# introlab/rtabmap

Measured on AMD Instinct MI355X. Metric: loop-closure candidates/sec (49k vocab, 100k signatures, 500 desc/frame), higher is better.
Workload: dtype f32; 1 GPU; SURF-64 fp32 brute-force 2-NN (49k words) + NNDR + TF-IDF likelihood (100000 signatures x 500 words, Zipf), 500 desc/frame, 1 frame/step; world_size_observed=1, collective_backend=none, parallelism=1 GPU, last_frame_top_candidate_ok=True

## Files before the change

rtabmap_amd/csrc/engine.h:

```cpp
#pragma once
#include <hip/hip_runtime.h>
#include <stdint.h>
#include <algorithm>
#include <chrono>
#include <cmath>
#include <deque>
#include <string>
#include <thread>
#include <unordered_map>
#include <vector>

#include "../../include/lcd.h"
#include "devbuf.h"
#include "lcd_kernels.h"
#include "bayes.h"
#include "tfidf.h"

struct RowMirror {
    std::vector<int32_t> h_row_key;
    std::vector<char> h_row_live;
    bool rows_sorted = true;
    std::unordered_map<int32_t, int32_t> word_row;
    bool word_row_valid = false;
    int32_t next_word_id = 1;
// ... 206 lines not shown
    lcd::DevBuf d_queries, d_partial, d_knn_row, d_knn_word, d_knn_wslot, d_knn_dist, d_selfdist, d_out_word, d_out_wslot,
        d_n_new, d_tmp_i32, d_extra_rows, d_extra_id, d_extra_word, d_extra_dist, d_extra_row, d_like, d_slots, d_bits, row_norm, norm_max, d_partial2, d_partial3, d_fail_list, d_fail_count;
    lcd::DevBuf d_shard_selfdist;
    const void* shard_sd_desc = nullptr; int shard_sd_q = 0;
    bool fail_count_clean = false;
    bool bf_family() const { return knn_mode == 2 || knn_mode == 3; }
    int f16() const { return knn_mode == 3 ? 1 : 0; }
    int knn_mode = 2;
    bool hamming_mfma = false;
    bool wide_mfma = false;
    lcd::DevBuf d_wide_norm;
    int pipeline = 0;
    hipStream_t kst = nullptr;
    FramePipeline pipe;
    const void* last_fail_count = nullptr;
    AppendLog applog;
    int64_t vocab_capacity_cfg = 0;
    int64_t tail_filled_rows = 0;
    lcd::DevBuf d_rmlog;
    int64_t rm_seen = 0;
    bool rm_pending = false;
    int frames_since_reconcile = 0;
    int enqueue_clean(const int32_t* reg_cnt = nullptr);
    int reconcile();
    int32_t shard_first = 0, shard_block = 0;
    int shard_append = 0;
    int filter_units = -1;
    int strip_tiles = 0;
    lcd::PipeOpts popt;
    int sync_all();
// ... 35 lines not shown
```

rtabmap_amd/csrc/engine.hip:

```cpp
#include "engine_impl.h"
#include <dlfcn.h>

#include <algorithm>
#include <chrono>
#include <cmath>
#include <cstdlib>
#include <cstring>
#include <new>
#include <numeric>
#include <unordered_map>

using namespace lcd;

static_assert(sizeof(lcd::HypothesisOut) == sizeof(lcd_hypothesis), "lcd_hypothesis is the kernel's output record");

int RowMirror::find(int32_t word_id) {
    if (rows_sorted) {
        auto it = std::lower_bound(h_row_key.begin(), h_row_key.end(), word_id);
        if (it == h_row_key.end() || *it != word_id) return -1;
        const int r = (int)(it - h_row_key.begin());
        return h_row_live[r] ? r : -1;
    }
    if (!word_row_valid) {
        word_row.clear();
// ... 308 lines not shown
                                       h->d_knn_word.as<int32_t>(), h->d_knn_dist.as<float>(), h->d_bits.as<uint32_t>(), bw));
    }
    r->q = q;
    r->flags = (incremental ? LCD_Q_INCREMENTAL : 0) | (together ? LCD_Q_NEW_WORDS_COMPARED : 0);
    r->nndr = nndr;
    r->have_index = have_index;
    r->knn_word = h->d_knn_word.as<int32_t>();
    r->knn_dist = h->d_knn_dist.as<float>();
    r->selfdist = together ? h->d_selfdist.as<float>() : nullptr;
    r->ld = ld;
    r->cand_bits = together ? h->d_bits.as<uint32_t>() : nullptr;
    r->bw = bw;
    r->out_word = d_out_word;
    r->out_n_new = h->d_n_new.as<int32_t>();
    r->knn_row = h->d_knn_row.as<int32_t>();
    r->row_wslot = h->row_wslot.as<int32_t>();
    r->out_wslot = d_out_wslot;
    r->new_ws = WsRuns();
    r->cand_list = nullptr; r->cand_cnt = nullptr;
    if (side) {
        CandBits lay;
        cand_bits_layout(lay, h->d_bits.as<uint32_t>(), q, bw);
        r->cand_list = lay.list; r->cand_cnt = lay.cnt;
    }
    r->fail_count = nullptr;
    return LCD_OK;
}

extern "C" {

// ... 1341 lines not shown
```

rtabmap_amd/csrc/frame_pipeline.hip:

```cpp
#include "engine_impl.h"

#include <algorithm>
#include <chrono>
#include <cstring>

using namespace lcd;

namespace {
struct FrameHostTimer {
    lcd_engine* h; std::chrono::steady_clock::time_point t0;
    explicit FrameHostTimer(lcd_engine* e) : h(e), t0(std::chrono::steady_clock::now()) {}
    ~FrameHostTimer() { h->frame_host_ns += std::chrono::duration_cast<std::chrono::nanoseconds>(std::chrono::steady_clock::now() - t0).count(); h->frame_calls += 1; }
};
struct HostLap {
    lcd_engine* h; std::chrono::steady_clock::time_point t;
    explicit HostLap(lcd_engine* e) : h(e), t(std::chrono::steady_clock::now()) {}
    void lap(int i) { const auto n = std::chrono::steady_clock::now(); h->host_prof[i] += std::chrono::duration_cast<std::chrono::nanoseconds>(n - t).count(); t = n; }
};
struct FrameShape { bool incremental, together; int ld, bw; };
inline FrameShape frame_shape(const lcd_frame_args& a) {
    const bool incremental = (a.flags & LCD_Q_INCREMENTAL) != 0;
    const int ld = (a.q + 63) / 64 * 64;
    return FrameShape{incremental, incremental && (a.flags & LCD_Q_NEW_WORDS_COMPARED) != 0, ld, ld / 32};
}
// ... 153 lines not shown
        LCD_HIP(h, ring_reserve_grow(h, f.set, &FramePipeline::FrameScratch::d_partial3, knn_rowpar_partial_bytes((int)rows3, q),
                                     f.chained ? knn_rowpar_partial_bytes((int)std::min<int64_t>(rows3 + rows3 / 2 + 65536, 0x7FFFFF00ll), q) : 0));
    }
    k.vocab = h->vocab.p; k.vocab_bf = h->vocab_bf.p; k.row_norm = h->row_norm.as<float>(); k.norm_max_bits = h->norm_max.as<uint32_t>();
    k.row_id = h->row_id.as<int32_t>(); k.queries = a.d_descriptors; k.partial = sc.d_partial2.p;
    k.qsplit = sc.d_qsplit.p; k.qnorm = sc.d_qnorm.as<float>();
    k.out_row = sc.d_knn_row.as<int32_t>(); k.out_word = sc.d_knn_word.as<int32_t>(); k.out_dist = sc.d_knn_dist.as<float>();
    k.fail_list = sc.d_fail_list.as<int32_t>(); k.fail_count = sc.d_fail_count.as<int32_t>();
    k.n_lo = nullptr; k.n_hi = nullptr;
    if (f.chained) { k.n_lo = h->applog.count_after(f.vseq); k.n_hi = h->applog.count_before(f.vseq); }
    k.cb = CandBits();
    if (together) { k.cb.selfdist = sc.d_selfdist.as<float>(); k.cb.ld = ld; k.cb.nq = q; k.cb.have_index = 1; cand_bits_layout(k.cb, sc.d_bits.as<uint32_t>(), q, bw); }
    if (!sc.fail_count_clean) LCD_HIP(h, hipMemsetAsync(sc.d_fail_count.p, 0, 8, h->stream));
    sc.fail_count_clean = true;
    h->last_fail_count = sc.d_fail_count.p;
    ResolveArgs& r = f.r;
    r = ResolveArgs();
    r.q = q; r.flags = (incremental ? LCD_Q_INCREMENTAL : 0) | (together ? LCD_Q_NEW_WORDS_COMPARED : 0); r.nndr = a.nndr_ratio; r.have_index = 1;
    r.knn_word = k.out_word; r.knn_dist = k.out_dist; r.selfdist = together ? sc.d_selfdist.as<float>() : nullptr; r.ld = ld;
    r.cand_bits = together ? sc.d_bits.as<uint32_t>() : nullptr; r.bw = bw; r.out_word = a.d_word_ids; r.out_n_new = h->d_n_new.as<int32_t>();
    r.cand_list = together ? k.cb.list : nullptr; r.cand_cnt = together ? k.cb.cnt : nullptr;
    r.knn_row = k.out_row; r.row_wslot = h->row_wslot.as<int32_t>(); r.out_wslot = sc.d_out_wslot.as<int32_t>(); r.new_ws = WsRuns();
    r.fail_count = sc.d_fail_count.as<int32_t>();
    RowparArgs& rp = r.rp;
    rp.enabled = 1; rp.vocab = (const float*)h->vocab.p; rp.row_id = h->row_id.as<int32_t>(); rp.n_rows = (int)rows_bound;
    rp.n_rows_dev = k.n_hi;
    rp.queries = (const float*)a.d_descriptors; rp.fail_list = sc.d_fail_list.as<int32_t>(); rp.partial = (unsigned long long*)sc.d_partial3.p;
    rp.out_row = k.out_row; rp.out_word = k.out_word; rp.out_dist = k.out_dist;
    if (together) rp.cb = k.cb;
    return LCD_OK;
// ... 237 lines not shown

int lcd_frame_dev(lcd_engine* h, const lcd_frame_args* a) {
    LCD_TRY
    LCD_CHECK_HANDLE(h);
    FrameHostTimer timer__(h);
    lcd_engine::Range range__(h, "lcd_frame_dev");
    LCD_DEV_NODRAIN(h);
    return frame_dev_body(h, a);
    LCD_CATCH(h)
}

int lcd_debug_host_profile(const lcd_engine* h, int64_t* out9) {
    if (!h || !out9) return LCD_ERR_INVALID;
    for (int i = 0; i < 9; ++i) out9[i] = h->host_prof[i];
    return LCD_OK;
}

int lcd_slot_count(const lcd_engine* h, int64_t* n_slots) {
    if (!h || !n_slots) return LCD_ERR_INVALID;
    *n_slots = h->tfidf.n_slots + h->pipe.owed_sigs();
    return LCD_OK;
}

int lcd_frame_host(lcd_engine* h, const lcd_frame_host_args* a) {
    LCD_TRY
    LCD_CHECK_HANDLE(h);
    lcd_engine::Range range__(h, "lcd_frame_host");
    LCD_DEV(h);
    if (!a || a->struct_size != (int32_t)sizeof(lcd_frame_host_args)) return h->fail(LCD_ERR_INVALID, "lcd_frame_host: bad argument block");
    const int q = a->q;
// ... 47 lines not shown
```

rtabmap_amd/csrc/frame_tail_body.cuh:

```cuda
#pragma once
#include "tfidf.h"
#include "resolve_body.cuh"
#include "rowpar_body.cuh"

namespace lcd {
namespace {

template <typename T> __device__ __forceinline__ T gload(const T* p) { return *(const __attribute__((address_space(1))) T*)p; }
__device__ __forceinline__ uint2 gload2(const uint2* p) {
    const unsigned long long v = *(const __attribute__((address_space(1))) unsigned long long*)p;
    return make_uint2((uint32_t)v, (uint32_t)(v >> 32));
}

__device__ __forceinline__ uint4 gload4(const uint4* p) {
    typedef uint32_t u32x4 __attribute__((ext_vector_type(4)));
    const u32x4 v = *(const __attribute__((address_space(1))) u32x4*)p;
    return make_uint4(v.x, v.y, v.z, v.w);
}

__device__ __forceinline__ int32_t idf_to_fixed(float idf) {
    float s = idf * 67108864.0f;
    s = fminf(fmaxf(s, -2147483520.0f), 2147483520.0f);
    return (int32_t)rintf(s);
}
// ... 383 lines not shown
    else { asm volatile("" : "+v"(n_in_early), "+v"(ne0));
           fmask = resolve_body<NT>(ft_dyn_smem, r.q, r.flags, r.nndr, r.have_index, r.knn_word, r.knn_dist, r.selfdist, r.ld, r.cand_bits, r.bw, r.out_word,
                                    r.out_n_new, r.knn_row, r.row_wslot, r.out_wslot, r.new_ws); }
    if (threadIdx.x == 0 && r.fail_count) { r.fail_count[0] = 0; r.fail_count[1] = 0; r.fail_count[3] = 0; }
    if (r.ap.enabled) append_new_rows<NT>(r.ap, r.q, fmask, ft_dyn_smem + 2 * ((r.q + 63) / 64 * 2), r.new_ws, ft_dyn_smem + 2 * a.H + a.H / 64 + 8 + r.q,
                                          nullptr, 0, n_in_early);
    else append_pass_on(r.ap);
    FT_STAMP(1);
    retire_body(retire, a.slot_begin, a.slot_cnt, a.nw, a.slot_ni, a.slot_sig);
    __syncthreads();
    FT_STAMP(2);
    frame_words_body<NT, true>(ft_dyn_smem, a, lds_ws, have_ne0, ne0);
    FT_STAMP(3);
}

template <int NT>
__device__ __forceinline__ void frame_resolve_part(uint32_t* ft_dyn_smem, const ResolveArgs& r, int wb, int n_wb) {
    if (wb > 0) { rowpar_body<64, NT>(r.rp, wb - 1, n_wb - 1, r.fail_count); return; }
    constexpr int KPT = 1024 / NT;
    const bool fast = r.q <= KPT * NT;
    const bool helpers = r.rp.enabled && n_wb > 1;
    if (helpers && !fast) {
        if (threadIdx.x == 0 && r.fail_count[0] > 0) {
            while (__hip_atomic_load(&r.fail_count[3], __ATOMIC_RELAXED, __HIP_MEMORY_SCOPE_AGENT) == 0) __builtin_amdgcn_s_sleep(8);
            __builtin_amdgcn_fence(__ATOMIC_ACQUIRE, "agent");
        }
        __syncthreads();
    }
    int n_in_early = -1;
    const int32_t* cnt_in = (r.ap.enabled && r.ap.cnt_in) ? r.ap.cnt_in : nullptr;
    if (!fast && cnt_in) n_in_early = gload(cnt_in);
    FT_STAMP(0);
    const uint32_t* fmask;
    if (fast) fmask = resolve_body_fast<NT, KPT>(ft_dyn_smem, nullptr, r.q, r.flags, r.nndr, r.have_index, r.knn_word, r.knn_dist, r.selfdist,
                                                 r.ld, r.cand_bits, r.bw, r.out_word, r.out_n_new, r.knn_row, r.row_wslot, r.out_wslot, r.new_ws,
                                                 r.cand_list, r.cand_cnt, &n_in_early, cnt_in, helpers ? r.fail_count : nullptr, r.slots_are_rows != 0, r.straight != 0);
    else { asm volatile("" : "+v"(n_in_early)); fmask = resolve_body<NT>(ft_dyn_smem, r.q, r.flags, r.nndr, r.have_index, r.knn_word, r.knn_dist, r.selfdist, r.ld, r.cand_bits, r.bw, r.out_word,
                                  r.out_n_new, r.knn_row, r.row_wslot, r.out_wslot, r.new_ws, r.slots_are_rows != 0); }
    if (threadIdx.x == 0 && r.fail_count) { r.fail_count[0] = 0; r.fail_count[1] = 0; r.fail_count[3] = 0; }
    if (r.ap.enabled && r.ap.defer_rows) append_publish<NT>(r.ap, r.q, fmask, ft_dyn_smem + 2 * ((r.q + 63) / 64 * 2), n_in_early);
    else if (r.ap.enabled) {
        const int used = (3 * ((r.q + 63) / 64 * 2) + 4 + r.q + 3) & ~3;
        const int rows = (r.ap.lds_bytes / 4 - used) / 64;
        append_new_rows<NT>(r.ap, r.q, fmask, ft_dyn_smem + 2 * ((r.q + 63) / 64 * 2), r.new_ws, ft_dyn_smem + 3 * ((r.q + 63) / 64 * 2) + 4,
                            reinterpret_cast<float*>(ft_dyn_smem + used), rows > 0 ? (rows & ~3) : 0, n_in_early);
    } else append_pass_on(r.ap);
    FT_STAMP(1);
}
template <int NT>
__device__ __forceinline__ void frame_register_part_keys(uint32_t* ft_dyn_smem, const FwArgs& a, const RetireArgs& retire) {
    uint32_t ne0 = 0u;
    const bool have_ne0 = a.do_register && a.ne_counter != nullptr;
    if (threadIdx.x == 0 && have_ne0) ne0 = gload(a.ne_counter);
// ... 82 lines not shown
```

rtabmap_amd/csrc/knn_mfma_kernels.hip:

```cpp
#include <hip/hip_ext.h>
#include "lcd_kernels.h"
#include "rowpar_body.cuh"
#include "shard_body.cuh"
#include "frame_tail_body.cuh"
#include "score_body.cuh"

#include <algorithm>
#include <cstdlib>

namespace lcd {
namespace {

typedef float f32x16 __attribute__((ext_vector_type(16)));
constexpr int MF_BLOCK = 256;
constexpr int MF_WAVES = 4;
constexpr int MF_KEEP = 4;

__global__ void row_norm_kernel(const float* __restrict__ vocab, const int32_t* __restrict__ row_id, int first, int n, int dim,
                                float* __restrict__ aug, uint32_t* __restrict__ norm_max_bits) {
    const int r = first + blockIdx.x * blockDim.x + threadIdx.x;
    if (r >= first + n) return;
    float s = __int_as_float(0x7f800000);
    if (row_id[r] != 0) {
        s = 0.0f;
// ... 889 lines not shown
        static const hipError_t attrp1 = hipFuncSetAttribute(reinterpret_cast<const void*>(&frame_a_kernel_p<1>),
                                                             hipFuncAttributeMaxDynamicSharedMemorySize, (int)BF_LDS_BYTES_P);
        (void)attrp0; (void)attrp1;
        auto kern = f16 ? frame_a_kernel_p<1> : frame_a_kernel_p<0>;
        if (timed) hipExtLaunchKernelGGL(kern, dim3(grid), dim3(PIPE_BLOCK), (uint32_t)BF_LDS_BYTES_P, s, ev_begin, ev_end, 0u, f, px, tr, r, a, ret, qs);
        else kern<<<grid, PIPE_BLOCK, BF_LDS_BYTES_P, s>>>(f, px, tr, r, a, ret, qs);
    } else {
        auto kern = f16 ? frame_a_kernel<1> : frame_a_kernel<0>;
        if (timed) hipExtLaunchKernelGGL(kern, dim3(grid), dim3(PIPE_BLOCK), (uint32_t)BF_LDS_BYTES_Q, s, ev_begin, ev_end, 0u, f, tr, r, a, ret, qs);
        else kern<<<grid, PIPE_BLOCK, BF_LDS_BYTES_Q, s>>>(f, tr, r, a, ret, qs);
    }
    return hipGetLastError();
}


hipError_t launch_frame_b(const PipeKnn* k, const ScoreArgs* score, int score_wgs, hipStream_t s, hipEvent_t ev_begin, hipEvent_t ev_end,
                          const AppendRowsArgs* app, const PipeOpts& opt) {
    RerankArgs rk{};
    int n_rerank = 0;
    if (k) {
        const MfmaPlan& p = k->plan;
        uint64_t* pk = (uint64_t*)k->partial;
        rk.pk = pk; rk.pl = (uint32_t*)(pk + (size_t)(p.n_blocks > 0 ? p.n_blocks : 1) * BF_KEEP * p.qpad);
        rk.n_blocks = p.n_blocks; rk.nq = p.q; rk.vocab = (const float*)k->vocab; rk.queries = (const float*)k->queries; rk.row_id = k->row_id;
        rk.norm_max_bits = k->norm_max_bits; rk.out_row = k->out_row; rk.out_word = k->out_word; rk.out_dist = k->out_dist;
        rk.fail_list = k->fail_list; rk.fail_count = k->fail_count; rk.cb = k->cb; rk.n_lo = k->n_lo; rk.n_hi = k->n_hi; rk.plan_rows = p.n_rows; rk.f16 = p.f16;
        n_rerank = ((p.q + 1) / 2 + 7) & ~7;
    }
    ScoreArgs A{};
    if (score) A = *score; else score_wgs = 0;
    AppendRowsArgs ar{};
    int n_app = 0;
    if (app && app->ap.enabled && app->ap.defer_rows) { ar = *app; n_app = ar.n_wgs = APPEND_ROW_WGS; }
    if (n_rerank + score_wgs + n_app == 0) return hipSuccess;
    const uint32_t dyn = ((k && k->n_hi) || n_app) ? PIPE_B_STAGE_ROWS * 256u + 512u : 0u;
    rk.stage_rows = (dyn && k && k->n_hi) ? (int)PIPE_B_STAGE_ROWS : 0;
    ar.ap.lds_bytes = (int)(PIPE_B_STAGE_ROWS * 256u);
    if (k && n_app) { rk.pend_desc = ar.ap.descriptors; rk.pend_list = ar.ap.list_out; rk.pend_first_id = ar.ap.first_id; }
    if (k && n_app && opt.cross_frames && k->cross && k->cross_cols == (const void*)ar.ap.descriptors) { rk.cross = k->cross; rk.cross_ld = k->cross_ld; }
    const bool writers = opt.append_from_rerank == 0;
    if (!writers && k && n_app > 0 && k->n_hi && k->plan.q > 0 && rk.stage_rows >= 4) n_app = 0;
    const bool shadow = k && k->plan.n_shadow > 0 && k->sh_mask && k->sh_x && k->sh_q > 0 && app && app->ap.enabled && app->ap.defer_rows && rk.pend_desc && !rk.cross;
    if (k && k->plan.n_shadow > 0 && !shadow) return hipErrorInvalidValue;
    if (shadow) { rk.sh_mask = k->sh_mask; rk.sh_q = k->sh_q; rk.sh_x = k->sh_x; rk.sh_ld = k->sh_ld; }
    const int n_wr = (!writers && n_app == 0 && k && app && app->ap.enabled && app->ap.defer_rows && k->n_hi && k->plan.q > 0 && rk.stage_rows >= 4 && !rk.cross &&
                      (opt.row_writer_wgs > 0 || shadow)) ? (opt.row_writer_wgs > 0 ? opt.row_writer_wgs : 16) : 0;
    if (shadow && n_wr == 0) return hipErrorInvalidValue;
    const bool split = n_app > 0 && score && score->n_closed >= (opt.append_split_buckets >= 0 ? opt.append_split_buckets : APPEND_SPLIT_BUCKETS);
    if (split || n_app == 0) {
        if (n_rerank + score_wgs > 0) {
            if (ev_begin != nullptr && ev_end != nullptr)
                hipExtLaunchKernelGGL(frame_b_kernel<false>, dim3(n_rerank + n_wr + score_wgs), dim3(PIPE_B_BLOCK), dyn, s, ev_begin, ev_end, 0u, rk, n_rerank, A, score_wgs, ar, n_wr);
            else frame_b_kernel<false><<<n_rerank + n_wr + score_wgs, PIPE_B_BLOCK, dyn, s>>>(rk, n_rerank, A, score_wgs, ar, n_wr);
        }
        if (n_app > 0) append_rows_kernel<<<n_app, PIPE_B_BLOCK, PIPE_B_STAGE_ROWS * 256u, s>>>(ar);
        return hipGetLastError();
    }
    if (ev_begin != nullptr && ev_end != nullptr)
        hipExtLaunchKernelGGL(frame_b_kernel<true>, dim3(n_rerank + score_wgs + n_app), dim3(PIPE_B_BLOCK), dyn, s, ev_begin, ev_end, 0u, rk, n_rerank, A, score_wgs, ar, 0);
    else frame_b_kernel<true><<<n_rerank + score_wgs + n_app, PIPE_B_BLOCK, dyn, s>>>(rk, n_rerank, A, score_wgs, ar, 0);
    return hipGetLastError();
}

}

extern "C" int lcd_debug_frame_plan(int q, int n_rows, int new_words_compared, int* out) {
    if (q <= 0 || n_rows <= 0 || !out) return -1;
    const int tiles = new_words_compared ? lcd::knn_selfdist_wgs(q) : 0;
    const lcd::MfmaPlan p = lcd::knn_bf16_plan_pipelined(q, n_rows, tiles, -1);
    out[0] = p.tiles_per_block; out[1] = p.n_blocks; out[2] = lcd::bf16_persistent_px(p); out[3] = tiles; out[4] = (q + lcd::BF_QB - 1) / lcd::BF_QB;
    return 0;
}

extern "C" int lcd_debug_wide_mfma_plan(int q, int n_rows, int dim, int units, int* out9) {
    lcd::WidePlan p;
    if (!out9 || !lcd::knn_wide_mfma_plan(q, n_rows, dim, units, &p)) return -1;
    out9[0] = p.tiles_per_block; out9[1] = p.n_blocks; out9[2] = p.n_qblocks; out9[3] = p.group_q; out9[4] = p.qpad;
    out9[5] = (int)(lcd::knn_wide_partial_bytes(p) / 4); out9[6] = lcd::MF_STRIP_TILES;
    out9[7] = (p.tiles_per_block + lcd::MF_STRIP_TILES - 1) / lcd::MF_STRIP_TILES; out9[8] = p.n_wgs;
    return 0;
// ... 18 lines not shown
```

rtabmap_amd/csrc/rerank_body.cuh:

```cuda

__device__ __forceinline__ float eps_bf16(int dim, float qn, float vn_max) {
    const float u = 5.9604645e-8f;
    return (3.1f * 1.5258789e-5f + ((3.0f * (float)dim + 4.0f) * 8.0f + 1.5f * (float)dim + 12.0f) * u) * 1.25f * (qn + vn_max);
}
__device__ __forceinline__ float eps_f16(int dim, float qn, float vn_max) {
    const float u = 5.9604645e-8f, u16 = 4.8828125e-4f;
    return ((2.0f * u16 + u16 * u16) + (((float)dim + 4.0f) * 8.0f + 1.5f * (float)dim + 12.0f) * u) * 1.25f * (qn + vn_max) +
           2.0f * (float)dim * 2.9802322e-8f * (2.0f + qn + vn_max);
}

__device__ __forceinline__ float eps_for(int dim, float qn, float vn_max) {
    return (3.5f * (float)dim + 16.0f) * 5.9604645e-8f * 1.25f * (qn + vn_max);
}

constexpr int RR_MAX_CAND = 128;
#ifdef LCD_B_TIMING
__device__ unsigned long long g_rr_timing[8 * 512];
#define RR_STAMP(i) do { if (threadIdx.x == 0 && blockIdx.x < 512) g_rr_timing[8 * blockIdx.x + (i)] = __builtin_amdgcn_s_memrealtime(); } while (0)
#else
#define RR_STAMP(i) do { } while (0)
#endif
__device__ __forceinline__ float l2_term4(const float4& v, const float4& q) {
    const float d0 = __fsub_rn(v.x, q.x), d1 = __fsub_rn(v.y, q.y), d2 = __fsub_rn(v.z, q.z), d3 = __fsub_rn(v.w, q.w);
    float t = __fmul_rn(d0, d0);
// ... 29 lines not shown
                                                     const float* __restrict__ pend_desc = nullptr, const uint32_t* __restrict__ pend_list = nullptr,
                                                     int32_t pend_first_id = 0
                                                     , const float* __restrict__ cross = nullptr, int cross_ld = 0
                                                     , const AppendRowsArgs& wr = AppendRowsArgs(), bool wr_on = false, int wr_index = 0, int wr_n = 1
                                                     , bool rows_only = false
                                                     , const uint32_t* __restrict__ sh_mask = nullptr, int sh_q = 0, const float* __restrict__ sh_x = nullptr, int sh_ld = 0
                                                     ) {
    static_assert(DIM == 64, "16 lanes x 4 floats per candidate row");
    constexpr int NT = HALVES * MF_BLOCK;
    int n_lo0 = 0, p_hi_ld = 0;
    if (pend_lo && pend_hi) asm volatile("s_load_dword %0, %2, 0x0\n\ts_load_dword %1, %3, 0x0\n\ts_waitcnt lgkmcnt(0)" : "=&s"(n_lo0), "=&s"(p_hi_ld) : "s"(pend_lo), "s"(pend_hi) : "memory");
    else { if (pend_lo) n_lo0 = pend_lo[0]; if (pend_hi) p_hi_ld = pend_hi[0]; }
    const int p_lo = pend_lo ? min(n_lo0, pend_cap) : 0, p_hi = p_hi_ld;
    const int32_t pend_id0 = pend_first_id > 0 ? pend_first_id : n_lo0 - pend_first_id;
    const int p_hi_s = sh_q > 0 ? min(p_hi, n_lo0) : p_hi;
    __shared__ uint32_t s_plist[NT];
    const uint32_t plreg = pend_list ? pend_list[threadIdx.x] : 0u;
    auto plist_at = [&](int j) -> uint32_t { return j < NT ? s_plist[j] : pend_list[j]; };
    constexpr int SH_MW_MAX = 128;
    __shared__ uint32_t s_shmask[2 * SH_MW_MAX + 1];
    const int sh_mw = sh_q > 0 ? (sh_q + 63) / 64 * 2 : 0;
    const uint32_t shreg = (sh_q > 0 && (int)threadIdx.x < 2 * sh_mw + 1) ? sh_mask[threadIdx.x] : 0u;
    auto sh_isword = [&](uint32_t j) -> bool { return (s_shmask[j >> 5] >> (j & 31)) & 1u; };
    auto sh_rank = [&](uint32_t j) -> int { return (int)(s_shmask[sh_mw + (j >> 5)] + (uint32_t)__popc(s_shmask[j >> 5] & ((1u << (j & 31)) - 1u))); };
    const int hf = HALVES == 2 ? (int)threadIdx.x / MF_BLOCK : 0;
    const int tid = HALVES == 2 ? (int)threadIdx.x % MF_BLOCK : (int)threadIdx.x, lane = tid & 63, wave = tid >> 6;
    auto stage_chunk = [&](int first, int n_chunk) {
        const int wv = (int)threadIdx.x >> 6, ln = (int)threadIdx.x & 63;
        const int n_inst = (n_chunk + 3) / 4;
        const int rot = (int)(((unsigned)blockIdx.x * 13u) % (unsigned)n_inst);
        auto issue = [&](auto list_at) {
            for (int i0 = wv; i0 < n_inst; i0 += HALVES * MF_WAVES) {
                const int i = i0 + rot < n_inst ? i0 + rot : i0 + rot - n_inst;
                stage_four_rows(stage, i, ln, n_chunk, [&](int rl) -> const float* {
                    const int r = first + rl;
                    return (pend_list && r >= n_lo0) ? pend_desc + (size_t)list_at(r - n_lo0) * DIM : vocab + (size_t)r * DIM;
                });
            }
        };
        if (!pend_list || first + n_chunk - n_lo0 <= NT) issue([&](int j) -> uint32_t { return s_plist[j]; });
// ... 12 lines not shown
        for (int j = wr_index + wr_n * ((int)threadIdx.x >> 4), m = (int)threadIdx.x >> 4; j < n_new; j += wr_n * (NT / 16), m += NT / 16) {
            const int rl = own ? m : n_lo0 + j - c0;
            if (rl < 0 || rl >= n_chunk) continue;
            const int32_t key = (c16 == 0 && wr.new_ws.n > 0) ? ws_runs_at_dev(wr.new_ws, j) : -1;
            const uint4 x = *reinterpret_cast<const uint4*>(staged_chunk(stage, rl, c16));
            append_write_row(ap, (size_t)n_lo0 + (size_t)j, c16, x, nmax);
            if (c16 == 0) {
                const size_t row = (size_t)n_lo0 + (size_t)j;
                ap.row_id[row] = ap.first_id > 0 ? ap.first_id + j : (int32_t)row - ap.first_id;
                ap.row_wslot[row] = key;
                if (key >= 0 && ap.wrow) ap.wrow[key] = (uint32_t)row + 1u;
            }
        }
        append_norm_max(ap, nmax);
    };
    auto store_mirror = [&]() {
        const AppendArgs& ap = wr.ap;
        if (ap.mirror_later && ap.host_mirror && wr_on && wr_index == 0 && threadIdx.x == 0)
            __hip_atomic_store(ap.host_mirror, ((unsigned long long)ap.tag << 32) | (unsigned long long)(uint32_t)p_hi, __ATOMIC_RELAXED, __HIP_MEMORY_SCOPE_SYSTEM);
    };

    if (rows_only) {
        const int n_new = p_hi - n_lo0;
        if (!wr_on || stage == nullptr || stage_rows < 4 || pend_list == nullptr || n_new <= wr_index) { store_mirror(); return; }
        s_plist[threadIdx.x] = plreg;
        lds_barrier();
        const int wv = (int)threadIdx.x >> 6, ln = (int)threadIdx.x & 63;
        const int n_mine = (n_new - wr_index + wr_n - 1) / wr_n;
        const int cap = stage_rows & ~3;
        for (int m0 = 0; m0 < n_mine; m0 += cap) {
            const int n_chunk = min(cap, n_mine - m0);
            if (m0 > 0) __syncthreads();
            for (int i = wv; i * 4 < n_chunk; i += HALVES * MF_WAVES)
                stage_four_rows(stage, i, ln, n_chunk, [&](int rl) -> const float* { return pend_desc + (size_t)plist_at(wr_index + wr_n * (m0 + rl)) * DIM; });
            asm volatile("s_waitcnt vmcnt(0)" ::: "memory");
            __syncthreads();
            {
                const AppendArgs& ap = wr.ap;
                const int c16 = (int)threadIdx.x & 15;
                float nmax = 0.0f;
// ... 28 lines not shown
    };
    auto bound_at = [&](int b) -> uint32_t { return BF16 ? partial_lmin[(size_t)b * qpad_t + qi] : partial_lmin[(size_t)qi * n_blocks + b]; };
    constexpr uint32_t INF = 0x7f800000u;
    __shared__ uint32_t s_a0_all[HALVES][MF_WAVES], s_a1_all[HALVES][MF_WAVES], s_bound_all[HALVES][MF_WAVES];
    __shared__ int s_ncand_all[HALVES];
    __shared__ uint64_t s_cand_all[HALVES][RR_MAX_CAND], s_exact_all[HALVES][RR_MAX_CAND];
    __shared__ int32_t s_word_all[HALVES][RR_MAX_CAND];
    __shared__ float s_err_all[HALVES][MF_WAVES];
    __shared__ uint64_t s_pend_all[HALVES][MF_WAVES][2];
    uint32_t (&s_a0)[MF_WAVES] = s_a0_all[hf]; uint32_t (&s_a1)[MF_WAVES] = s_a1_all[hf]; uint32_t (&s_bound)[MF_WAVES] = s_bound_all[hf];
    int& s_ncand = s_ncand_all[hf];
    uint64_t (&s_cand)[RR_MAX_CAND] = s_cand_all[hf]; uint64_t (&s_exact)[RR_MAX_CAND] = s_exact_all[hf];
    int32_t (&s_word)[RR_MAX_CAND] = s_word_all[hf];
    float (&s_err)[MF_WAVES] = s_err_all[hf];
    uint64_t (&s_pend)[MF_WAVES][2] = s_pend_all[hf];

    RR_STAMP(0);
    const uint64_t kreg0 = tid < n_keys ? key_at(tid) : KEY_NONE;
    const uint64_t kreg1 = tid + MF_BLOCK < n_keys ? key_at(tid + MF_BLOCK) : KEY_NONE;
    const uint64_t kreg2 = tid + 2 * MF_BLOCK < n_keys ? key_at(tid + 2 * MF_BLOCK) : KEY_NONE;
    const uint32_t breg0 = tid < n_blocks ? bound_at(tid) : INF;
    const float4 q4 = reinterpret_cast<const float4*>(queries + (size_t)qi * DIM)[lane & 15];
    const float vn_max = __uint_as_float(norm_max_bits[0]);
    float dreg0 = __int_as_float(0x7f800000), dreg1 = __int_as_float(0x7f800000);
    if (cb.bits) {
        if (tid < cb.nq) dreg0 = cb.selfdist[(size_t)qi * cb.ld + tid];
        if (tid + MF_BLOCK < cb.nq) dreg1 = cb.selfdist[(size_t)qi * cb.ld + tid + MF_BLOCK];
    }
    float2 xsh = make_float2(__int_as_float(0x7f800000), __int_as_float(0x7f800000));
    if (sh_q > 0 && 2 * tid < sh_ld) xsh = *reinterpret_cast<const float2*>(sh_x + (size_t)qi * sh_ld + 2 * tid);
    float qn = fmaf(q4.w, q4.w, fmaf(q4.z, q4.z, fmaf(q4.y, q4.y, q4.x * q4.x)));
#pragma unroll
    for (int m = 8; m >= 1; m >>= 1) qn += __shfl_xor(qn, m, 64);

    uint32_t a0 = INF, a1 = INF, bound = breg0;
    auto see = [&](uint64_t key, int c) {
        const uint32_t sc = min((uint32_t)(key >> 32), INF);
        if (LAST_KEY_BOUNDS && (c % KEEP) == KEEP - 1) bound = min(bound, sc);
        const uint32_t h = max(a0, sc);
        a0 = min(a0, sc);
        a1 = min(a1, h);
    };
    see(kreg0, tid);
    see(kreg1, tid + MF_BLOCK);
    see(kreg2, tid + 2 * MF_BLOCK);
// ... 15 lines not shown
        lds_barrier();
    }
    if (staged) stage_chunk(p_lo, min(stage_rows, p_hi_s - p_lo));
    if (use_cross) {
        const int wv = (int)threadIdx.x >> 6, ln = (int)threadIdx.x & 63;
        for (int i = wv; i * 4 < n_own; i += HALVES * MF_WAVES)
            stage_four_rows(stage, i, ln, n_own, [&](int rl) -> const float* { return pend_desc + (size_t)plist_at(wr_index + wr_n * rl) * DIM; });
        const int n_pend = p_hi - p_lo;
        const float* crow = cross + (size_t)qi * cross_ld;
        for (int j0 = 0; j0 < n_pend; j0 += MF_BLOCK) {
            const float* src = crow + plist_at(min(j0 + tid, n_pend - 1));
            __builtin_amdgcn_global_load_lds((const __attribute__((address_space(1))) void*)src,
                                             (__attribute__((address_space(3))) void*)(xd + hf * XD_MAX + j0 + wave * 64), 4, 0, 0);
        }
    }
    if (staged && lane < 16 && wave == 0) reinterpret_cast<float4*>(stage + (size_t)stage_rows * DIM)[hf * 16 + lane] = q4;
    lds_barrier();
    RR_STAMP(1);
    a0 = s_a0[0]; a1 = s_a1[0]; bound = s_bound[0];
#pragma unroll
    for (int wi = 1; wi < MF_WAVES; ++wi) {
        const uint32_t o0 = s_a0[wi], o1 = s_a1[wi];
        a1 = min(max(a0, o0), min(a1, o1));
        a0 = min(a0, o0);
        bound = min(bound, s_bound[wi]);
    }
    const float eps = BF16 ? (f16 ? eps_f16(DIM, qn, vn_max) : eps_bf16(DIM, qn, vn_max)) : eps_for(DIM, qn, vn_max);
    const float tau = __uint_as_float(a1);
    const float thr = tau + (2.0f * eps + tau * 3.0517578e-5f);

    auto take = [&](uint64_t key) {
        const uint32_t sc = (uint32_t)(key >> 32);
        if (key != KEY_NONE && sc < INF && __uint_as_float(sc) <= thr) {
            const int slot = atomicAdd(&s_ncand, 1);
            if (slot < RR_KEYS) s_cand[slot] = key;
        }
    };
    take(kreg0);
    take(kreg1);
    take(kreg2);
// ... 28 lines not shown
            const uint32_t row = cand_row(i);
            const bool sh = sh_q > 0 && (uint32_t)key >= SHADOW_ROW_BASE;
            const uint32_t sj = (uint32_t)key - SHADOW_ROW_BASE;
            const bool in_range = sh ? (GS == 1 || (i & 3) == 0) : (GS == 1 || row < row_limit);
            const uint32_t rrow = in_range ? row : (uint32_t)key;
            const float* src = sh ? pend_desc + (size_t)sj * DIM : vocab + (size_t)rrow * DIM;
            v4 = reinterpret_cast<const float4*>(src)[lane & 15];
            wid = 0;
            if ((lane & 15) == 0) wid = sh ? pend_id0 + sh_rank(sj) : row_id[rrow];
        };
        auto finish = [&](int i, const float4& v4, int32_t wid) {
            const uint64_t key = s_cand[GS == 4 ? (i >> 2) : i];
            const uint32_t row = cand_row(i);
            const bool sh = sh_q > 0 && (uint32_t)key >= SHADOW_ROW_BASE;
            const bool in_range = sh ? (GS == 1 || (i & 3) == 0) : (GS == 1 || row < row_limit);
            const float t = l2_term4(v4, q4);
            float res = 0.0f;
#pragma unroll
            for (int j = 0; j < 16; ++j) res = __fadd_rn(res, __shfl(t, (lane & 48) + j, 64));
            const bool live = in_range && (GS == 1 || __shfl(wid, lane & 48, 64) != 0);
            if (!live) res = __int_as_float(0x7f800000);
            float gmin = res;
            if (GS == 4) { gmin = fminf(gmin, __shfl_xor(gmin, 16, 64)); gmin = fminf(gmin, __shfl_xor(gmin, 32, 64)); }
            if ((lane & 15) == 0) {
                s_exact[i] = live ? (((uint64_t)__float_as_uint(res) << 32) | (uint32_t)i) : KEY_NONE;
                s_word[i] = wid;
                if (gmin < __int_as_float(0x7f800000)) err_ratio = fmaxf(err_ratio, fabsf(__uint_as_float((uint32_t)(key >> 32)) - gmin) / eps);
            }
        };
        constexpr int STEP = MF_BLOCK / 16;
        int i = tid >> 4;
// ... 14 lines not shown
    {
        uint64_t pb = KEY_NONE, ps = KEY_NONE;
        constexpr int PU = 4;
        if (use_cross) {
            asm volatile("s_waitcnt vmcnt(0)" ::: "memory");
            RR_STAMP(4);
            for (int j = tid; j < p_hi - p_lo; j += MF_BLOCK)
                top2_push(pb, ps, ((uint64_t)__float_as_uint(xd[hf * XD_MAX + j]) << 32) | (uint32_t)(p_lo + j));
        } else if (staged) {
            for (int c0 = p_lo; c0 < p_hi_s; c0 += stage_rows) {
                const int n_chunk = min(stage_rows, p_hi_s - c0);
                if (c0 > p_lo) { __syncthreads(); stage_chunk(c0, n_chunk); }
                asm volatile("s_waitcnt vmcnt(0)" ::: "memory");
                __syncthreads();
                RR_STAMP(4);
                const float4* sq = reinterpret_cast<const float4*>(stage + (size_t)stage_rows * DIM) + hf * 16;
                for (int r = tid; r < n_chunk; r += MF_BLOCK) {
                    float res = 0.0f;
#pragma unroll 4
                    for (int c = 0; c < 16; ++c) res = __fadd_rn(res, l2_term4(*staged_chunk(stage, r, c), sq[c]));
                    top2_push(pb, ps, ((uint64_t)__float_as_uint(res) << 32) | (uint32_t)(c0 + r));
                }
                if (wr_on && sh_q == 0 && c0 + stage_rows < p_hi) write_rows(c0, n_chunk);
            }
        } else
        for (int base = p_lo; base < (pend_list ? min(p_hi_s, n_lo0) : p_hi_s); base += PU * (MF_BLOCK / 16)) {
            float4 v4[PU];
#pragma unroll
            for (int u = 0; u < PU; ++u) {
                const int r0 = base + u * (MF_BLOCK / 16) + (tid >> 4);
                v4[u] = reinterpret_cast<const float4*>(vocab + (size_t)min(r0, p_hi_s - 1) * DIM)[lane & 15];
            }
#pragma unroll
            for (int u = 0; u < PU; ++u) {
                const int r0 = base + u * (MF_BLOCK / 16) + (tid >> 4);
                const float t = l2_term4(v4[u], q4);
                float res = 0.0f;
#pragma unroll
                for (int j = 0; j < 16; ++j) res = __fadd_rn(res, __shfl(t, (lane & 48) + j, 64));
                if ((lane & 15) == 0 && r0 < p_hi_s) top2_push(pb, ps, ((uint64_t)__float_as_uint(res) << 32) | (uint32_t)r0);
            }
        }
        if (p_hi_s > p_lo) {
            wave_top2_reduce(pb, ps);
            if (lane == 0) { s_pend[wave][0] = pb; s_pend[wave][1] = ps; }
        }
    }
    RR_STAMP(5);
    lds_barrier();
    RR_STAMP(6);
    asm volatile("" : "+v"(dreg0), "+v"(dreg1));
// ... 23 lines not shown
                if (key == second) ssecond = i;
            }
#pragma unroll
        for (int m = 32; m >= 1; m >>= 1) {
            sbest = max(sbest, __shfl_xor(sbest, m, 64));
            ssecond = max(ssecond, __shfl_xor(ssecond, m, 64));
        }
#ifdef LCD_RR_SUBSTAMP
        RR_STAMP(5);
#endif
    }
    if (tid == 0) s_thr = (cb.have_index && second != KEY_NONE) ? __uint_as_float((uint32_t)(second >> 32)) : __int_as_float(0x7f800000);

    if (tid == 0 && valid) {
        err_ratio = fmaxf(fmaxf(s_err[0], s_err[1]), fmaxf(s_err[2], s_err[3]));
        const uint64_t win[2] = {best, second};
        const int sl[2] = {sbest, ssecond};
        int32_t wout[2] = {0, 0};
#pragma unroll
        for (int j = 0; j < 2; ++j) {
            if (win[j] == KEY_NONE) continue;
            const int32_t rw = (int32_t)(uint32_t)win[j];
            wout[j] = sl[j] >= 0 ? s_word[sl[j]] : ((pend_list && rw >= n_lo0) ? pend_id0 + (rw - n_lo0) : row_id[rw]);
        }
        bool ok = !overflow;
        if (ok && bound < INF) {
            if (second == KEY_NONE) ok = false;
            else ok = __uint_as_float(bound) - eps > __uint_as_float((uint32_t)(second >> 32));
        }
        if (err_ratio >= 0.5f) ok = false;
// ... 50 lines not shown
```

rtabmap_amd/synth.py:

```python
import numpy as np


def vocab_surf(n, seed=49000, dim=64):
    rng = np.random.default_rng(seed)
    v = rng.standard_normal((n, dim), dtype=np.float32)
    v4 = v.reshape(n, dim // 4, 4)
    v4[:, :, 2] = np.abs(v4[:, :, 2]) + np.abs(v4[:, :, 0])
    v4[:, :, 3] = np.abs(v4[:, :, 3]) + np.abs(v4[:, :, 1])
    v /= np.linalg.norm(v, axis=1, keepdims=True)
    return np.ascontiguousarray(v, dtype=np.float32)


def queries_surf(vocab, q, seed=500, frac_known=0.7, sigma=0.05):
    rng = np.random.default_rng(seed)
    n, dim = vocab.shape
    out = np.empty((q, dim), np.float32)
    known = rng.random(q) < frac_known
    src = rng.integers(0, n, q)
    noise = rng.standard_normal((q, dim), dtype=np.float32) * np.float32(sigma)
    fresh = vocab_surf(q, seed=seed + 7919, dim=dim)
    out[known] = vocab[src[known]] + noise[known]
    out[~known] = fresh[~known]
    out /= np.linalg.norm(out, axis=1, keepdims=True)
    return np.ascontiguousarray(out, dtype=np.float32)


def vocab_orb(n, seed=200000, nbytes=32):
    rng = np.random.default_rng(seed)
    return rng.integers(0, 256, (n, nbytes), dtype=np.uint8)


def queries_orb(vocab, q, seed=501, frac_known=0.7, flip=0.1):
    rng = np.random.default_rng(seed)
    n, nb = vocab.shape
    known = rng.random(q) < frac_known
    src = rng.integers(0, n, q)
    out = rng.integers(0, 256, (q, nb), dtype=np.uint8)
    flips = np.packbits(rng.random((q, nb * 8)) < flip, axis=1)
# ... 48 lines not shown
```

Before: 3.346 billion candidates/s.

## Move rerank query vector into LDS, defer loads, scalarize resolve pointers, add debug hooks

The rerank kernel now keeps the query float4 in a small shared-memory array instead of the staging buffer tail, which removes 512 bytes from the dynamic LDS request. Loads of the pending list and shadow mask are deferred to where they are used. The early-exit check for rows-only writers moves ahead of those loads, and the bound reduction is folded into the final thread-0 step. Resolve pointers are forced into scalar registers and the half index uses readfirstlane, both meant to lower VGPR pressure. The change also adds debug entry points for kNN readback and launch-route counters, plus a synthetic revisit generator.

After: 3.394 billion candidates/s (median of 6 runs). +1.4%, better.

```diff
diff --git a/rtabmap_amd/csrc/engine.h b/rtabmap_amd/csrc/engine.h
--- a/rtabmap_amd/csrc/engine.h
+++ b/rtabmap_amd/csrc/engine.h
@@ -244,6 +244,7 @@
     hipStream_t kst = nullptr;
     FramePipeline pipe;
     const void* last_fail_count = nullptr;
+    const void* dbg_knn_row = nullptr; const void* dbg_knn_word = nullptr; const void* dbg_knn_dist = nullptr; int dbg_knn_q = 0;
     AppendLog applog;
     int64_t vocab_capacity_cfg = 0;
     int64_t tail_filled_rows = 0;
diff --git a/rtabmap_amd/csrc/engine.hip b/rtabmap_amd/csrc/engine.hip
--- a/rtabmap_amd/csrc/engine.hip
+++ b/rtabmap_amd/csrc/engine.hip
@@ -346,6 +346,7 @@
     r->out_word = d_out_word;
     r->out_n_new = h->d_n_new.as<int32_t>();
     r->knn_row = h->d_knn_row.as<int32_t>();
+    h->dbg_knn_row = h->d_knn_row.p; h->dbg_knn_word = h->d_knn_word.p; h->dbg_knn_dist = h->d_knn_dist.p; h->dbg_knn_q = q;
     r->row_wslot = h->row_wslot.as<int32_t>();
     r->out_wslot = d_out_wslot;
     r->new_ws = WsRuns();
diff --git a/rtabmap_amd/csrc/frame_pipeline.hip b/rtabmap_amd/csrc/frame_pipeline.hip
--- a/rtabmap_amd/csrc/frame_pipeline.hip
+++ b/rtabmap_amd/csrc/frame_pipeline.hip
@@ -191,6 +191,7 @@
     if (!sc.fail_count_clean) LCD_HIP(h, hipMemsetAsync(sc.d_fail_count.p, 0, 8, h->stream));
     sc.fail_count_clean = true;
     h->last_fail_count = sc.d_fail_count.p;
+    h->dbg_knn_row = k.out_row; h->dbg_knn_word = k.out_word; h->dbg_knn_dist = k.out_dist; h->dbg_knn_q = q;
     ResolveArgs& r = f.r;
     r = ResolveArgs();
     r.q = q; r.flags = (incremental ? LCD_Q_INCREMENTAL : 0) | (together ? LCD_Q_NEW_WORDS_COMPARED : 0); r.nndr = a.nndr_ratio; r.have_index = 1;
@@ -458,6 +459,26 @@
     if (!h || !out9) return LCD_ERR_INVALID;
     for (int i = 0; i < 9; ++i) out9[i] = h->host_prof[i];
     return LCD_OK;
+}
+
+int lcd_debug_last_frame_knn(lcd_engine* h, int32_t* out_row, int32_t* out_word, float* out_dist, int capacity, int* out_q, int* out_rejected) {
+    LCD_TRY
+    LCD_CHECK_HANDLE(h);
+    LCD_DEV_NODRAIN(h);
+    if (!out_q) return LCD_ERR_INVALID;
+    *out_q = h->dbg_knn_q;
+    if (out_rejected) *out_rejected = 0;
+    if (h->dbg_knn_q <= 0 || !h->dbg_knn_row) return LCD_OK;
+    if (capacity < h->dbg_knn_q) return h->fail(LCD_ERR_INVALID, "lcd_debug_last_frame_knn: capacity below the frame's descriptor count");
+    LCD_HIP(h, hipStreamSynchronize(h->stream));
+    if (h->kst && h->kst != h->stream) LCD_HIP(h, hipStreamSynchronize(h->kst));
+    const size_t bytes = (size_t)h->dbg_knn_q * 2 * 4;
+    if (out_row) LCD_HIP(h, hipMemcpy(out_row, h->dbg_knn_row, bytes, hipMemcpyDeviceToHost));
+    if (out_word) LCD_HIP(h, hipMemcpy(out_word, h->dbg_knn_word, bytes, hipMemcpyDeviceToHost));
+    if (out_dist) LCD_HIP(h, hipMemcpy(out_dist, h->dbg_knn_dist, bytes, hipMemcpyDeviceToHost));
+    if (out_rejected && h->last_fail_count) LCD_HIP(h, hipMemcpy(out_rejected, h->last_fail_count, 4, hipMemcpyDeviceToHost));
+    return LCD_OK;
+    LCD_CATCH(h)
 }
 
 int lcd_slot_count(const lcd_engine* h, int64_t* n_slots) {
diff --git a/rtabmap_amd/csrc/frame_tail_body.cuh b/rtabmap_amd/csrc/frame_tail_body.cuh
--- a/rtabmap_amd/csrc/frame_tail_body.cuh
+++ b/rtabmap_amd/csrc/frame_tail_body.cuh
@@ -421,9 +421,19 @@
     FT_STAMP(3);
 }
 
+template <class T>
+__device__ __forceinline__ T* scalar_global(T* p) {
+    auto g = (__attribute__((address_space(1))) T*)p;
+    asm volatile("" : "+s"(g));
+    return (T*)g;
+}
+
 template <int NT>
 __device__ __forceinline__ void frame_resolve_part(uint32_t* ft_dyn_smem, const ResolveArgs& r, int wb, int n_wb) {
     if (wb > 0) { rowpar_body<64, NT>(r.rp, wb - 1, n_wb - 1, r.fail_count); return; }
+    int32_t* const out_word = scalar_global(r.out_word); int32_t* const out_n_new = scalar_global(r.out_n_new); int32_t* const out_wslot = scalar_global(r.out_wslot);
+    const int32_t* const knn_row = scalar_global(r.knn_row); const int32_t* const row_wslot = scalar_global(r.row_wslot);
+    const uint2* const cand_list = scalar_global(r.cand_list); const int32_t* const cand_cnt = scalar_global(r.cand_cnt);
     constexpr int KPT = 1024 / NT;
     const bool fast = r.q <= KPT * NT;
     const bool helpers = r.rp.enabled && n_wb > 1;
@@ -440,10 +450,10 @@
     FT_STAMP(0);
     const uint32_t* fmask;
     if (fast) fmask = resolve_body_fast<NT, KPT>(ft_dyn_smem, nullptr, r.q, r.flags, r.nndr, r.have_index, r.knn_word, r.knn_dist, r.selfdist,
-                                                 r.ld, r.cand_bits, r.bw, r.out_word, r.out_n_new, r.knn_row, r.row_wslot, r.out_wslot, r.new_ws,
-                                                 r.cand_list, r.cand_cnt, &n_in_early, cnt_in, helpers ? r.fail_count : nullptr, r.slots_are_rows != 0, r.straight != 0);
-    else { asm volatile("" : "+v"(n_in_early)); fmask = resolve_body<NT>(ft_dyn_smem, r.q, r.flags, r.nndr, r.have_index, r.knn_word, r.knn_dist, r.selfdist, r.ld, r.cand_bits, r.bw, r.out_word,
-                                  r.out_n_new, r.knn_row, r.row_wslot, r.out_wslot, r.new_ws, r.slots_are_rows != 0); }
+                                                 r.ld, r.cand_bits, r.bw, out_word, out_n_new, knn_row, row_wslot, out_wslot, r.new_ws,
+                                                 cand_list, cand_cnt, &n_in_early, cnt_in, helpers ? r.fail_count : nullptr, r.slots_are_rows != 0, r.straight != 0);
+    else { asm volatile("" : "+v"(n_in_early)); fmask = resolve_body<NT>(ft_dyn_smem, r.q, r.flags, r.nndr, r.have_index, r.knn_word, r.knn_dist, r.selfdist, r.ld, r.cand_bits, r.bw, out_word,
+                                  out_n_new, knn_row, row_wslot, out_wslot, r.new_ws, r.slots_are_rows != 0); }
     if (threadIdx.x == 0 && r.fail_count) { r.fail_count[0] = 0; r.fail_count[1] = 0; r.fail_count[3] = 0; }
     if (r.ap.enabled && r.ap.defer_rows) append_publish<NT>(r.ap, r.q, fmask, ft_dyn_smem + 2 * ((r.q + 63) / 64 * 2), n_in_early);
     else if (r.ap.enabled) {
diff --git a/rtabmap_amd/csrc/knn_mfma_kernels.hip b/rtabmap_amd/csrc/knn_mfma_kernels.hip
--- a/rtabmap_amd/csrc/knn_mfma_kernels.hip
+++ b/rtabmap_amd/csrc/knn_mfma_kernels.hip
@@ -927,6 +927,7 @@
 }
 
 
+static long long g_b_routes[8];
 hipError_t launch_frame_b(const PipeKnn* k, const ScoreArgs* score, int score_wgs, hipStream_t s, hipEvent_t ev_begin, hipEvent_t ev_end,
                           const AppendRowsArgs* app, const PipeOpts& opt) {
     RerankArgs rk{};
@@ -946,7 +947,7 @@
     int n_app = 0;
     if (app && app->ap.enabled && app->ap.defer_rows) { ar = *app; n_app = ar.n_wgs = APPEND_ROW_WGS; }
     if (n_rerank + score_wgs + n_app == 0) return hipSuccess;
-    const uint32_t dyn = ((k && k->n_hi) || n_app) ? PIPE_B_STAGE_ROWS * 256u + 512u : 0u;
+    const uint32_t dyn = ((k && k->n_hi) || n_app) ? PIPE_B_STAGE_ROWS * 256u : 0u;
     rk.stage_rows = (dyn && k && k->n_hi) ? (int)PIPE_B_STAGE_ROWS : 0;
     ar.ap.lds_bytes = (int)(PIPE_B_STAGE_ROWS * 256u);
     if (k && n_app) { rk.pend_desc = ar.ap.descriptors; rk.pend_list = ar.ap.list_out; rk.pend_first_id = ar.ap.first_id; }
@@ -959,6 +960,11 @@
     const int n_wr = (!writers && n_app == 0 && k && app && app->ap.enabled && app->ap.defer_rows && k->n_hi && k->plan.q > 0 && rk.stage_rows >= 4 && !rk.cross &&
                       (opt.row_writer_wgs > 0 || shadow)) ? (opt.row_writer_wgs > 0 ? opt.row_writer_wgs : 16) : 0;
     if (shadow && n_wr == 0) return hipErrorInvalidValue;
+    if (k && n_rerank > 0) {
+        g_b_routes[0] += 1; g_b_routes[1] += shadow ? 1 : 0; g_b_routes[2] += n_wr > 0 ? 1 : 0; g_b_routes[3] += rk.cross ? 1 : 0;
+        g_b_routes[4] += (rk.pend_list && !shadow && !rk.cross && rk.stage_rows >= 4) ? 1 : 0;
+        g_b_routes[5] += (!writers && n_app == 0 && n_wr == 0 && rk.pend_list) ? 1 : 0; g_b_routes[6] = n_wr; g_b_routes[7] = n_rerank;
+    }
     const bool split = n_app > 0 && score && score->n_closed >= (opt.append_split_buckets >= 0 ? opt.append_split_buckets : APPEND_SPLIT_BUCKETS);
     if (split || n_app == 0) {
         if (n_rerank + score_wgs > 0) {
@@ -977,6 +983,12 @@
 
 }
 
+extern "C" int lcd_debug_launch_b_routes(long long* out8, int reset) {
+    if (out8) for (int i = 0; i < 8; ++i) out8[i] = lcd::g_b_routes[i];
+    if (reset) for (int i = 0; i < 8; ++i) lcd::g_b_routes[i] = 0;
+    return 0;
+}
+
 extern "C" int lcd_debug_frame_plan(int q, int n_rows, int new_words_compared, int* out) {
     if (q <= 0 || n_rows <= 0 || !out) return -1;
     const int tiles = new_words_compared ? lcd::knn_selfdist_wgs(q) : 0;
diff --git a/rtabmap_amd/csrc/rerank_body.cuh b/rtabmap_amd/csrc/rerank_body.cuh
--- a/rtabmap_amd/csrc/rerank_body.cuh
+++ b/rtabmap_amd/csrc/rerank_body.cuh
@@ -67,16 +67,21 @@
     const int p_lo = pend_lo ? min(n_lo0, pend_cap) : 0, p_hi = p_hi_ld;
     const int32_t pend_id0 = pend_first_id > 0 ? pend_first_id : n_lo0 - pend_first_id;
     const int p_hi_s = sh_q > 0 ? min(p_hi, n_lo0) : p_hi;
+    auto store_mirror = [&]() {
+        const AppendArgs& ap = wr.ap;
+        if (ap.mirror_later && ap.host_mirror && wr_on && wr_index == 0 && threadIdx.x == 0)
+            __hip_atomic_store(ap.host_mirror, ((unsigned long long)ap.tag << 32) | (unsigned long long)(uint32_t)p_hi, __ATOMIC_RELAXED, __HIP_MEMORY_SCOPE_SYSTEM);
+    };
+    if (rows_only && (!wr_on || stage == nullptr || stage_rows < 4 || pend_list == nullptr || p_hi - n_lo0 <= wr_index)) { store_mirror(); return; }
     __shared__ uint32_t s_plist[NT];
-    const uint32_t plreg = pend_list ? pend_list[threadIdx.x] : 0u;
+    uint32_t plreg = 0u, shreg = 0u;
     auto plist_at = [&](int j) -> uint32_t { return j < NT ? s_plist[j] : pend_list[j]; };
     constexpr int SH_MW_MAX = 128;
     __shared__ uint32_t s_shmask[2 * SH_MW_MAX + 1];
     const int sh_mw = sh_q > 0 ? (sh_q + 63) / 64 * 2 : 0;
-    const uint32_t shreg = (sh_q > 0 && (int)threadIdx.x < 2 * sh_mw + 1) ? sh_mask[threadIdx.x] : 0u;
     auto sh_isword = [&](uint32_t j) -> bool { return (s_shmask[j >> 5] >> (j & 31)) & 1u; };
     auto sh_rank = [&](uint32_t j) -> int { return (int)(s_shmask[sh_mw + (j >> 5)] + (uint32_t)__popc(s_shmask[j >> 5] & ((1u << (j & 31)) - 1u))); };
-    const int hf = HALVES == 2 ? (int)threadIdx.x / MF_BLOCK : 0;
+    const int hf = HALVES == 2 ? __builtin_amdgcn_readfirstlane((int)threadIdx.x / MF_BLOCK) : 0;
     const int tid = HALVES == 2 ? (int)threadIdx.x % MF_BLOCK : (int)threadIdx.x, lane = tid & 63, wave = tid >> 6;
     auto stage_chunk = [&](int first, int n_chunk) {
         const int wv = (int)threadIdx.x >> 6, ln = (int)threadIdx.x & 63;
@@ -119,16 +124,10 @@
         }
         append_norm_max(ap, nmax);
     };
-    auto store_mirror = [&]() {
-        const AppendArgs& ap = wr.ap;
-        if (ap.mirror_later && ap.host_mirror && wr_on && wr_index == 0 && threadIdx.x == 0)
-            __hip_atomic_store(ap.host_mirror, ((unsigned long long)ap.tag << 32) | (unsigned long long)(uint32_t)p_hi, __ATOMIC_RELAXED, __HIP_MEMORY_SCOPE_SYSTEM);
-    };
 
     if (rows_only) {
         const int n_new = p_hi - n_lo0;
-        if (!wr_on || stage == nullptr || stage_rows < 4 || pend_list == nullptr || n_new <= wr_index) { store_mirror(); return; }
-        s_plist[threadIdx.x] = plreg;
+        s_plist[threadIdx.x] = pend_list[threadIdx.x];
         lds_barrier();
         const int wv = (int)threadIdx.x >> 6, ln = (int)threadIdx.x & 63;
         const int n_mine = (n_new - wr_index + wr_n - 1) / wr_n;
@@ -187,6 +186,8 @@
     int32_t (&s_word)[RR_MAX_CAND] = s_word_all[hf];
     float (&s_err)[MF_WAVES] = s_err_all[hf];
     uint64_t (&s_pend)[MF_WAVES][2] = s_pend_all[hf];
+    __shared__ float4 s_q_all[HALVES][16];
+    const float4* const s_q = s_q_all[hf];
 
     RR_STAMP(0);
     const uint64_t kreg0 = tid < n_keys ? key_at(tid) : KEY_NONE;
@@ -202,6 +203,8 @@
     }
     float2 xsh = make_float2(__int_as_float(0x7f800000), __int_as_float(0x7f800000));
     if (sh_q > 0 && 2 * tid < sh_ld) xsh = *reinterpret_cast<const float2*>(sh_x + (size_t)qi * sh_ld + 2 * tid);
+    if (pend_list) plreg = pend_list[threadIdx.x];
+    if (sh_q > 0 && (int)threadIdx.x < 2 * sh_mw + 1) shreg = sh_mask[threadIdx.x];
     float qn = fmaf(q4.w, q4.w, fmaf(q4.z, q4.z, fmaf(q4.y, q4.y, q4.x * q4.x)));
 #pragma unroll
     for (int m = 8; m >= 1; m >>= 1) qn += __shfl_xor(qn, m, 64);
@@ -247,16 +250,15 @@
                                              (__attribute__((address_space(3))) void*)(xd + hf * XD_MAX + j0 + wave * 64), 4, 0, 0);
         }
     }
-    if (staged && lane < 16 && wave == 0) reinterpret_cast<float4*>(stage + (size_t)stage_rows * DIM)[hf * 16 + lane] = q4;
+    if (lane < 16 && wave == 0) s_q_all[hf][lane] = q4;
     lds_barrier();
     RR_STAMP(1);
-    a0 = s_a0[0]; a1 = s_a1[0]; bound = s_bound[0];
+    a0 = s_a0[0]; a1 = s_a1[0];
 #pragma unroll
     for (int wi = 1; wi < MF_WAVES; ++wi) {
         const uint32_t o0 = s_a0[wi], o1 = s_a1[wi];
         a1 = min(max(a0, o0), min(a1, o1));
         a0 = min(a0, o0);
-        bound = min(bound, s_bound[wi]);
     }
     const float eps = BF16 ? (f16 ? eps_f16(DIM, qn, vn_max) : eps_bf16(DIM, qn, vn_max)) : eps_for(DIM, qn, vn_max);
     const float tau = __uint_as_float(a1);
@@ -315,7 +317,7 @@
             const uint32_t row = cand_row(i);
             const bool sh = sh_q > 0 && (uint32_t)key >= SHADOW_ROW_BASE;
             const bool in_range = sh ? (GS == 1 || (i & 3) == 0) : (GS == 1 || row < row_limit);
-            const float t = l2_term4(v4, q4);
+            const float t = l2_term4(v4, s_q[lane & 15]);
             float res = 0.0f;
 #pragma unroll
             for (int j = 0; j < 16; ++j) res = __fadd_rn(res, __shfl(t, (lane & 48) + j, 64));
@@ -360,11 +362,10 @@
                 asm volatile("s_waitcnt vmcnt(0)" ::: "memory");
                 __syncthreads();
                 RR_STAMP(4);
-                const float4* sq = reinterpret_cast<const float4*>(stage + (size_t)stage_rows * DIM) + hf * 16;
                 for (int r = tid; r < n_chunk; r += MF_BLOCK) {
                     float res = 0.0f;
 #pragma unroll 4
-                    for (int c = 0; c < 16; ++c) res = __fadd_rn(res, l2_term4(*staged_chunk(stage, r, c), sq[c]));
+                    for (int c = 0; c < 16; ++c) res = __fadd_rn(res, l2_term4(*staged_chunk(stage, r, c), s_q[c]));
                     top2_push(pb, ps, ((uint64_t)__float_as_uint(res) << 32) | (uint32_t)(c0 + r));
                 }
                 if (wr_on && sh_q == 0 && c0 + stage_rows < p_hi) write_rows(c0, n_chunk);
@@ -380,7 +381,7 @@
 #pragma unroll
             for (int u = 0; u < PU; ++u) {
                 const int r0 = base + u * (MF_BLOCK / 16) + (tid >> 4);
-                const float t = l2_term4(v4[u], q4);
+                const float t = l2_term4(v4[u], s_q[lane & 15]);
                 float res = 0.0f;
 #pragma unroll
                 for (int j = 0; j < 16; ++j) res = __fadd_rn(res, __shfl(t, (lane & 48) + j, 64));
@@ -434,6 +435,8 @@
 
     if (tid == 0 && valid) {
         err_ratio = fmaxf(fmaxf(s_err[0], s_err[1]), fmaxf(s_err[2], s_err[3]));
+        static_assert(MF_WAVES == 4, "the four waves' partial results");
+        bound = min(min(s_bound[0], s_bound[1]), min(s_bound[2], s_bound[3]));
         const uint64_t win[2] = {best, second};
         const int sl[2] = {sbest, ssecond};
         int32_t wout[2] = {0, 0};
diff --git a/rtabmap_amd/synth.py b/rtabmap_amd/synth.py
--- a/rtabmap_amd/synth.py
+++ b/rtabmap_amd/synth.py
@@ -22,6 +22,17 @@
     out[known] = vocab[src[known]] + noise[known]
     out[~known] = fresh[~known]
     out /= np.linalg.norm(out, axis=1, keepdims=True)
+    return np.ascontiguousarray(out, dtype=np.float32)
+
+
+def revisit_surf(rng, history, q, fresh_frac=0.3, sigma=0.02):
+    fresh = vocab_surf(q, seed=int(rng.integers(1 << 30)))
+    src = history[int(rng.integers(len(history)))]
+    out = src[rng.integers(0, src.shape[0], q)].copy()
+    out += rng.standard_normal(out.shape).astype(np.float32) * np.float32(sigma)
+    out /= np.linalg.norm(out, axis=1, keepdims=True)
+    m = rng.random(q) < fresh_frac
+    out[m] = fresh[m]
     return np.ascontiguousarray(out, dtype=np.float32)
 
 
```
